# NCAR/icar

Measured on AMD Instinct MI355X. Metric: grid-cell updates/sec (advection+microphysics), higher is better.
Workload: dtype f32; 1 GPU; 512x512x40 global grid, mpdata order-2+FCT advection of 9 scalars + thompson microphysics, ideal hill case (SURVEY 8d); decomposition=1x1, backend=none, ranks_seen=1, halo_check=not applicable (one image, no process group), mpdata_arithmetic=fused kernel (<= 1e-5 of the local scale per step)

## Files before the change

### icar_amd/csrc/ctx.h

```cpp
#pragma once
#include <hip/hip_runtime.h>
#include <string>
#include <map>
#include <vector>
#include "../../include/icar_hip.h"

#define ICAR_MAX_ADV 12

struct Dims {
    int nx, nz, ny;
    int sk, sj;
    __host__ __device__ inline int idx(int i, int k, int j) const { return i + nx * (k + nz * j); }
};

struct VarPtrs { float *p[ICAR_MAX_ADV]; };
struct CVarPtrs { const float *p[ICAR_MAX_ADV]; };

struct TimingGroup { double total_ms = 0; int launches = 0; };

struct ThompsonTables;
struct LinWinds;
struct Wsm3State;
struct Wsm6State;
struct IcarComm;


struct IcarStepState {
    bool configured = false;
    icar_hip_step_config cfg;
    std::vector<float> dz_levels;
    double model_time = 0.0;
    double mp_last_model_time = -999.0;
    int winds_scheme = 0, winds_dens = 0; float winds_dt = 0.f;
    float *h_val = nullptr;
    bool early_open = false, early_wreal = false, early_face = false;
    bool failed = false;
    bool winds_first = true;
};

enum { MPC_AU = 0, MPC_CUV, MPC_CUW, MPC_AV, MPC_CVU, MPC_CVW, MPC_AW, MPC_CWU, MPC_CWV, MPC_GH, MPC_GV, MPC_N };

struct icar_hip_ctx {
    int device = 0;
    int ims, ime, kms, kme, jms, jme;
    Dims d;
    size_t n3 = 0;
    hipStream_t stream = nullptr;
    bool own_stream = false;
    hipStream_t aux = nullptr, main_saved = nullptr;
    hipEvent_t ev_fork = nullptr, ev_join = nullptr;
    bool on_aux = false;
    void *field[ICAR_N_FIELDS] = {nullptr};
    float *dqdt[ICAR_N_FIELDS] = {nullptr};
    float *U = nullptr, *V = nullptr, *W = nullptr, *Wdz = nullptr;
    float *mpc = nullptr;
    int mpc_dens = -1;
    float *alt[ICAR_N_ADVECTABLE] = {nullptr};
    float *mpx_buf = nullptr;
    int mpx_nv = 0;
    int mpdata_exact = 0;
    bool winds_valid = false;
    unsigned long long wind_version = 0;
    bool wind_ptr_escaped = false;
    struct { bool valid = false, reduced = false; unsigned long long ver = 0; float dx = 0.f; std::vector<float> dzl; } cfl_pre;
    float *h_cfl_pre = nullptr;
    bool cfl_wait_failed = false;
    hipEvent_t cfl_ev = nullptr;
    float *iw_adj = nullptr;
    float *wgr_tmp = nullptr;
    float *d_red = nullptr;
    std::vector<float> dzl_host;
    int *d_flag = nullptr;
    ThompsonTables *thompson = nullptr;
    LinWinds *linwinds = nullptr;
    Wsm3State *wsm3 = nullptr;
    Wsm6State *wsm6 = nullptr;
    IcarComm *comm = nullptr;
    IcarStepState step;
    bool timing = false;
    std::string timing_only;
    std::vector<hipEvent_t> event_pool;
    std::map<std::string, TimingGroup> timers;
    std::vector<std::pair<std::string, std::pair<hipEvent_t, hipEvent_t>>> pending;
};

void icar_set_error(const std::string &msg);
int icar_hip_check(hipError_t e, const char *what);
#define HIPCHK(x) do { if (icar_hip_check((x), #x)) return 1; } while (0)

size_t icar_field_count(const icar_hip_ctx *c, int field);
float *icar_field_f(icar_hip_ctx *c, int field, bool required = true);

struct ScopedTimer {
    icar_hip_ctx *c; const char *group; hipEvent_t e0 = nullptr, e1 = nullptr;
    ScopedTimer(icar_hip_ctx *c_, const char *g);
    ~ScopedTimer();
};

int icar_advect_setup_winds(icar_hip_ctx *c, int scheme, float dt, float dx, int advect_density, bool with_wreal = false, bool *wreal_done = nullptr);
int icar_advect_run(icar_hip_ctx *c, int scheme, int order, int fct, int advect_density, const int *fields, int n);
int icar_mp_simple_run(icar_hip_ctx *c, float dt, int its, int ite, int jts, int jte, int kts, int kte, int *err);
int icar_mp_simple_run_tiles(icar_hip_ctx *c, float dt, int ntiles, const int tiles[][4], int kts, int kte, int *err);
int icar_mp_run(icar_hip_ctx *c, double dt_in, int halo, int subset);
int icar_update_dt(icar_hip_ctx *c, double *seconds);
int icar_substep(icar_hip_ctx *c, double dt, bool enforce);
int icar_halo_pack(icar_hip_ctx *c, int dir, int halo, const int *fields, int n, float *buf, bool unpack);
int icar_halo_pack_dirs(icar_hip_ctx *c, int ndir, const int *dirs, int halo, const int *fields, int n, void *const *bufs, bool unpack);
int icar_max_courant_run(icar_hip_ctx *c, float dx, const float *dz_levels, float *out, float *d_out);
int icar_max_abs_winds_run(icar_hip_ctx *c, float *out3);
int icar_balance_uvw_run(icar_hip_ctx *c, float dx, int update);
int icar_iterative_winds_correct_w(icar_hip_ctx *c, int update);
int icar_mass_conservative_acceleration(icar_hip_ctx *c, int update);
int icar_iterative_winds_sweep(icar_hip_ctx *c, float dx, int nsweeps, int update);
int icar_make_winds_grid_relative(icar_hip_ctx *c, int update);
int icar_box_copy(icar_hip_ctx *c, int field, int which, int i0, int ni, int j0, int nj, float *buf, bool unpack);
enum { ICAR_DIAG_CELL = 4, ICAR_DIAG_FACE = 8 };
int icar_diagnostic_update_run(icar_hip_ctx *c, int parts);
int icar_max_courant_prefetch_run(icar_hip_ctx *c, float dx, const float *dz_levels, bool allreduce);
bool icar_cfl_prefetched_global(icar_hip_ctx *c, float dx, const float *dz_levels, float *value);
bool icar_cfl_prefetch_waiting(icar_hip_ctx *c);
inline void icar_winds_changed(icar_hip_ctx *c) { c->winds_valid = false; ++c->wind_version; }
int icar_apply_forcing_run(icar_hip_ctx *c, double dt, const int *fields, const int *fb, int n, int w, int e, int s, int nn);
int icar_enforce_limits_run(icar_hip_ctx *c, const int *fields, int n);
int icar_thompson_init_run(icar_hip_ctx *c, const float *params, const int *flags);
int icar_thompson_run(icar_hip_ctx *c, float dt, int its, int ite, int jts, int jte, int kts, int kte,
                      int ids, int ide, int jds, int jde, int kds, int kde);
int icar_thompson_run_tiles(icar_hip_ctx *c, float dt, int ntiles, const int (*tiles)[4], int kts, int kte,
                            int ids, int ide, int jds, int jde, int kds, int kde);
int icar_thompson_prepare_constants(icar_hip_ctx *c);
void icar_thompson_free(icar_hip_ctx *c);
void icar_linwinds_free(icar_hip_ctx *c);
void icar_wsm3_free(icar_hip_ctx *c);
int icar_wsm3_init_run(icar_hip_ctx *c);
int icar_wsm3_run(icar_hip_ctx *c, float dt, int its, int ite, int jts, int jte, int kts, int kte);
void icar_wsm6_free(icar_hip_ctx *c);
int icar_wsm6_init_run(icar_hip_ctx *c);
int icar_wsm6_run(icar_hip_ctx *c, float dt, int its, int ite, int jts, int jte, int kts, int kte);
int icar_wsm6_run_tiles(icar_hip_ctx *c, float dt, int ntiles, const int tiles[][4], int kts, int kte);
int icar_linwinds_setup_run(icar_hip_ctx *c, const icar_hip_lt_options *o, const float *terrain, int nxg, int nyg, int ids, int jds, float dx);
int icar_linear_perturbation_run(icar_hip_ctx *c, float U, float V, float Nsq, float zb, float zt, float minimum_step, double *u_out, double *v_out);
int icar_linwinds_build_lut_run(icar_hip_ctx *c, const float *zb, const float *zt, int nlev);
int icar_linwinds_build_lut_varying_run(icar_hip_ctx *c, const float *zb3, const float *zt3, int nlev);
int icar_linwinds_lut_copy(icar_hip_ctx *c, int comp, float *host, int to_dev);
int icar_linwinds_lut_entry(icar_hip_ctx *c, int comp, int k, int i, int j, float *host);
int icar_linwinds_pert_copy(icar_hip_ctx *c, int comp, float *host, int to_dev);
int icar_linwinds_terrain_frequency(icar_hip_ctx *c, double *out, size_t cap, int *fnx, int *fny);
int icar_spatial_winds_run(icar_hip_ctx *c, int update);
int icar_thompson_table_download(icar_hip_ctx *c, const char *name, double *out, size_t cap, size_t *n_out);
```

### icar_amd/csrc/mpdata.hip

```cpp
#include "ctx.h"
#include <algorithm>
#include <cmath>
#include <type_traits>

#define MP_HL 3
#define MP_XOUT (64 - 2 * MP_HL)
#define MP_NW 8
#define MP_KB 5
#define MP_ZH 2
#define EPSQ 1e-10f
#define EPSF 1e-15f
#define HEPSQ 0.5e-10f

__device__ __forceinline__ float dpp_l(float x)
{ return __int_as_float(__builtin_amdgcn_mov_dpp(__float_as_int(x), 0x138, 0xf, 0xf, true)); }
__device__ __forceinline__ float dpp_r(float x)
{ return __int_as_float(__builtin_amdgcn_mov_dpp(__float_as_int(x), 0x130, 0xf, 0xf, true)); }
__device__ __forceinline__ float dpp_l2(float x, float o)
{ return __int_as_float(__builtin_amdgcn_update_dpp(__float_as_int(o), __float_as_int(x), 0x138, 0xf, 0xf, true)); }
__device__ __forceinline__ float dpp_r2(float x, float o)
{ return __int_as_float(__builtin_amdgcn_update_dpp(__float_as_int(o), __float_as_int(x), 0x130, 0xf, 0xf, true)); }
__device__ __forceinline__ float opaque(float x) { asm volatile("" : "+v"(x)); return x; }
__device__ __forceinline__ float frcp(float x) { return __builtin_amdgcn_rcpf(x); }
__device__ __forceinline__ float upw(float l, float r, float U) { return U * (U > 0.0f ? l : r); }
__device__ __forceinline__ float exact_quot(float a, float g, float &r)
{
    const float r0 = frcp(g);
    r = __builtin_fmaf(__builtin_fmaf(-g, r0, 1.0f), r0, r0);
    const float y = opaque(a * r);
    return __builtin_fmaf(__builtin_fmaf(-g, y, a), r, y);
}
__device__ __forceinline__ float max3f(float a, float b, float c) { return fmaxf(fmaxf(a, b), c); }
__device__ __forceinline__ float min3f(float a, float b, float c) { return fminf(fminf(a, b), c); }
using rsrc_t = __amdgpu_buffer_rsrc_t;
__device__ __forceinline__ rsrc_t mkrsrc(const float *p) { return __builtin_amdgcn_make_buffer_rsrc((void *)p, 0, -1, 0x00020000); }
__device__ __forceinline__ float ldb(rsrc_t r, int voff, int soff) { return __builtin_bit_cast(float, __builtin_amdgcn_raw_buffer_load_b32(r, voff, soff, 0)); }
__device__ __forceinline__ void stb(rsrc_t r, int voff, int soff, float v) { __builtin_amdgcn_raw_buffer_store_b32(__builtin_bit_cast(int, v), r, voff, soff, 0); }
template <bool RHO>
__global__ void __launch_bounds__(256)
k_mpdata_coef(Dims d, const float *__restrict__ U, const float *__restrict__ V, const float *__restrict__ Wz, const float *__restrict__ rho,
              const float *__restrict__ jaco, const float *__restrict__ dz, float *__restrict__ C)
{
    const size_t n3 = (size_t)d.nx * d.nz * d.ny;
    const int i = blockIdx.x * 64 + threadIdx.x, k = blockIdx.y * 4 + threadIdx.y, j = blockIdx.z;
    if (i >= d.nx || k >= d.nz) return;
    const int nx = d.nx, nz = d.nz, ny = d.ny;
    const int iL = max(i - 1, 0), iR = min(i + 1, nx - 1), jP = max(j - 1, 0), jN = min(j + 1, ny - 1), kB = max(k - 1, 0), kT = min(k + 1, nz - 1);
    auto at = [&](int ii, int kk, int jj) { return ii + nx * (kk + nz * jj); };
    auto G = [&](int ii, int kk, int jj) { const int c = at(ii, kk, jj); return RHO ? jaco[c] * rho[c] : jaco[c]; };
    const int c = at(i, k, j);
    const bool xin = (i > 0) && (i < nx - 1), kin = (k > 0) && (k < nz - 1);
    const float g = G(i, k, j), dzc = dz[c];
    {
        const float rG = frcp(g + G(iL, k, j));
        const float evv = (V[c] + V[at(i, k, jN)]) + (V[at(iL, k, j)] + V[at(iL, k, jN)]);
        const float evw = (Wz[c] + Wz[at(i, kB, j)]) + (Wz[at(iL, k, j)] + Wz[at(iL, kB, j)]);
        const float Uc = U[c], aU = fabsf(Uc), c0 = 0.0625f * Uc * rG;
        C[MPC_AU * n3 + c] = 0.5f * aU * (1.0f - 2.0f * aU * rG); C[MPC_CUV * n3 + c] = c0 * evv; C[MPC_CUW * n3 + c] = kin ? c0 * evw : 0.0f;
    }
    {
        const float rG = frcp(g + G(i, k, jP));
        const float evu = (U[at(i, k, jP)] + U[c]) + (U[at(iR, k, jP)] + U[at(iR, k, j)]);
        const float evw = (Wz[at(i, k, jP)] + Wz[at(i, kB, jP)]) + (Wz[c] + Wz[at(i, kB, j)]);
        const float Vc = V[c], aV = fabsf(Vc), c0 = 0.0625f * Vc * rG;
        C[MPC_AV * n3 + c] = 0.5f * aV * (1.0f - 2.0f * aV * rG); C[MPC_CVU * n3 + c] = xin ? c0 * evu : 0.0f; C[MPC_CVW * n3 + c] = kin ? c0 * evw : 0.0f;
    }
    if (k < nz - 1) {
        const float rG = frcp(g + G(i, kT, j));
        const float evu = (U[c] + U[at(i, kT, j)]) + (U[at(iR, k, j)] + U[at(iR, kT, j)]);
        const float evv = (V[c] + V[at(i, k, jN)]) + (V[at(i, kT, j)] + V[at(i, kT, jN)]);
        const float Wc = Wz[c], aW = fabsf(Wc), c0 = 0.0625f * Wc * rG;
        C[MPC_AW * n3 + c] = 0.5f * aW * (1.0f - 2.0f * aW * rG) * dzc; C[MPC_CWU * n3 + c] = xin ? c0 * evu * dzc : 0.0f; C[MPC_CWV * n3 + c] = c0 * evv * dzc;
    } else { C[MPC_AW * n3 + c] = 0.f; C[MPC_CWU * n3 + c] = 0.f; C[MPC_CWV * n3 + c] = 0.f; }
    const float gh = g, gv = RHO ? (dzc * jaco[c]) * rho[c] : dzc * jaco[c];
    C[MPC_GH * n3 + c] = gh; C[MPC_GV * n3 + c] = gv;
}

template <bool ST, int PAR> struct MpMode { static constexpr bool steady = ST; static constexpr int par = PAR; };

template <int KB, bool FCT, bool PASS1, bool EXACT>
__global__ void __launch_bounds__(64 * MP_NW) __attribute__((amdgpu_num_vgpr(124)))
k_mpdata_fused(Dims d, CVarPtrs qin, VarPtrs qout,
               const float *__restrict__ Ug, const float *__restrict__ Vg, const float *__restrict__ Wg,
               const float *__restrict__ Cg, unsigned asz, int clen, int ntile, int nchunk, int nscal, int nkr, int kstore)
{
    constexpr int H = KB + 2;
    __shared__ float s_q2[2][MP_NW][2][64];
    __shared__ float s_bz[2][MP_NW][4][64];
    constexpr int NW2 = MP_NW + 2;
    __shared__ int s_sync[3 * NW2 + 64];
    constexpr int NA4 = (H + 3) / 4, NB4 = 2 * KB;
    __shared__ float4 s_park[NA4 + NB4][64 * MP_NW];
    constexpr int NG4 = (KB + 3) / 4;
    __shared__ float4 s_rv[2][NG4][64 * MP_NW];

    const int lane = threadIdx.x;
    const int wv = __builtin_amdgcn_readfirstlane(threadIdx.y), nw = blockDim.y;
    const int tid = lane + 64 * wv;
    const int nx = d.nx, nz = d.nz, ny = d.ny;
    const int sj4 = 4 * d.sj;
    int tile, chunk, m, kr;
    {
        const unsigned id = blockIdx.x, nv = (unsigned)nscal, nitem = (unsigned)(ntile * nchunk * nkr) * nv;
        const unsigned cap = (nitem + 7u) / 8u, xcd = id & 7u, slot = id >> 3;
        const unsigned it = xcd * cap + slot;
        if (slot >= cap || it >= nitem) return;
        for (int t = tid; t < 2 * NW2; t += 64 * nw) { const int j = t % NW2; s_sync[t] = (j == 0 || j > nw) ? 0x7fffffff : 0; }
        __syncthreads();
        const unsigned g = it / nv;
        m = (int)(it - g * nv);
        tile = (int)(g % (unsigned)ntile); chunk = (int)((g / (unsigned)ntile) % (unsigned)nchunk); kr = (int)(g / (unsigned)(ntile * nchunk));
    }
    const int ka = kr * kstore, kb = min(ka + kstore - 1, nz - 1), kbase = max(ka - MP_ZH, 0);
    const float *__restrict__ qp = qin.p[0];
    float *__restrict__ outp = qout.p[0];
#pragma unroll
    for (int mm = 1; mm < ICAR_MAX_ADV; ++mm) if (mm == m) { qp = qin.p[mm]; outp = qout.p[mm]; }
    const rsrc_t q = mkrsrc(qp), out = mkrsrc(outp), Ur = mkrsrc(Ug), Vr = mkrsrc(Vg), Wr = mkrsrc(Wg),
                 cr = mkrsrc(Cg);

    const int i = 1 - MP_HL + tile * MP_XOUT + lane;
    const int ic = min(max(i, 0), nx - 1);
    const bool xin = (i > 0) && (i < nx - 1), xring = (i == 0) || (i == nx - 1);
    const bool lane_store = ((lane >= MP_HL) && (lane < 64 - MP_HL) && xin) || xring;
    float rm = (i <= 0 || i >= nx - 1) ? 0.0f : 1.0f;
    const int ja = 1 + chunk * clen, jb = min(ja + clen - 1, ny - 2);
    const int k0 = kbase + wv * KB;
    int vk[H];
#pragma unroll
    for (int h = 0; h < H; ++h) { vk[h] = 4 * ic + min(max(k0 - 1 + h, 0), nz - 1) * nx * 4; asm volatile("" : "+v"(vk[h])); }
    asm volatile("" : "+v"(rm));
    const float gmul = __int_as_float(__builtin_amdgcn_readfirstlane((k0 == 0) ? 0 : 0x3f800000));
    const bool topwave = (k0 + KB == nz);
    const int htop_u = __builtin_amdgcn_readfirstlane(nz - k0), kst0_u = __builtin_amdgcn_readfirstlane(ka - k0), kst1_u = __builtin_amdgcn_readfirstlane(kb - k0);
    const int wlo = max(wv - 1, 0), whi = min(wv + 1, nw - 1);
    const int q2lo = (wv > 0) ? 1 : 0, q2hi = (wv < nw - 1) ? 0 : 1;
    const int bzlo = (wv > 0) ? 2 : 0, bzhi = (wv < nw - 1) ? 0 : 2;
    int *const fpost = (lane == 0) ? &s_sync[1 + wv] : &s_sync[2 * NW2 + lane];
    int seqA = 0, seqB = 0;
#define MP_POST(e, seq)                                                                                                   \
    {                                                                                                                      \
        ++seq;                                                                                                             \
        __hip_atomic_store(fpost + (e) * NW2, seq, __ATOMIC_RELEASE, __HIP_MEMORY_SCOPE_WORKGROUP);                         \
    }
#define MP_WAIT(e, seq)                                                                                                    \
    {                                                                                                                      \
        int spin = 0;                                                                                                      \
        for (;;) {                                                                                                         \
            const int fa = __hip_atomic_load(&s_sync[(e) * NW2 + wv], __ATOMIC_ACQUIRE, __HIP_MEMORY_SCOPE_WORKGROUP);      \
            const int fb = __hip_atomic_load(&s_sync[(e) * NW2 + wv + 2], __ATOMIC_ACQUIRE, __HIP_MEMORY_SCOPE_WORKGROUP);  \
            if (__builtin_amdgcn_readfirstlane(min(fa, fb)) >= seq) break;                                                 \
            __builtin_amdgcn_s_sleep(1);                                                                                   \
            if (++spin > (1 << 26)) __builtin_trap();                        \
        }                                                                                                                  \
    }

#define LDQ(h, po) ldb(q, vk[h], (po))
#define LDC(a, h, po) ldb(cr, vk[h], (int)((unsigned)(a) * asz + (unsigned)(po)))
#define CLAMPJ(p) min(max((p), 0), ny - 1)

    struct QBuf { float v[H]; };
    struct PSet {
        float q2[H];
        float m[KB], n[KB];
        float Dx[KB], Sx[KB], Dz[KB], Sz[KB];
        float Fyd[KB];
        float rh[KB];
        float mh0, nh0, mh1, nh1;
    };
    QBuf Q0, Q1;
    PSet S0, S1;
#pragma unroll
    for (int kk = 0; kk < KB; ++kk) { S0.m[kk] = S0.n[kk] = 0.f; S0.Dx[kk] = S0.Sx[kk] = S0.Dz[kk] = S0.Sz[kk] = 0.f; S0.Fyd[kk] = 0.f; S0.rh[kk] = 0.f; }
#pragma unroll
    for (int h = 0; h < H; ++h) S0.q2[h] = 0.f;
    S0.mh0 = 0.f; S0.nh0 = 0.f; S0.mh1 = 0.f; S0.nh1 = 0.f;
    S1 = S0;
#pragma unroll
    for (int t = 0; t < NA4 + NB4; ++t) s_park[t][tid] = make_float4(0.f, 0.f, 0.f, 0.f);
#pragma unroll
    for (int t = 0; t < 2 * NG4; ++t) s_rv[t / NG4][t % NG4][tid] = make_float4(0.f, 0.f, 0.f, 0.f);
    const int P0 = ja - 3;
    float WN[KB + 1], UN[KB], VNN[KB], ghN[KB], gvN[KB];
#define ISSUE_LOADS_A(oN_, oNN_)                                                                                         \
    {                                                                                                                    \
        _Pragma("unroll") for (int h = 0; h <= KB; ++h) WN[h] = ldb(Wr, vk[h], (oN_));                                   \
        _Pragma("unroll") for (int kk = 0; kk < KB; ++kk) { UN[kk] = ldb(Ur, vk[kk + 1], (oN_)); VNN[kk] = ldb(Vr, vk[kk + 1], (oNN_)); } \
        _Pragma("unroll") for (int kk = 0; kk < KB; ++kk) { ghN[kk] = LDC(MPC_GH, kk + 1, (oN_)); gvN[kk] = LDC(MPC_GV, kk + 1, (oN_)); } \
    }
    {
        const int o0 = CLAMPJ(P0) * sj4, o1 = CLAMPJ(P0 + 1) * sj4, o2 = CLAMPJ(P0 + 2) * sj4;
        float qP0[KB], V1[KB];
#pragma unroll
        for (int kk = 0; kk < KB; ++kk) { qP0[kk] = LDQ(kk + 1, o0); V1[kk] = ldb(Vr, vk[kk + 1], o1); }
#pragma unroll
        for (int h = 0; h < H; ++h) Q0.v[h] = LDQ(h, o1);
#pragma unroll
        for (int h = 0; h < H; ++h) Q1.v[h] = LDQ(h, o2);
        ISSUE_LOADS_A(o1, o2)
        if (PASS1) {
#pragma unroll
            for (int kk = 0; kk < KB; ++kk) S0.Fyd[kk] = opaque(upw(qP0[kk], Q0.v[kk + 1], V1[kk]));
        }
    }
    auto step = [&](auto md, QBuf &qN, QBuf &qNN, PSet &sP, PSet &sN, const int P) {
        constexpr bool STEADY = decltype(md)::steady;
        const int par = STEADY ? decltype(md)::par : ((P - P0) & 1);
        const int N = P + 1;
        const bool haveN = STEADY || ((N >= 0) && (N <= ny - 1));
        const int oP = (STEADY ? P : CLAMPJ(P)) * sj4, oN = (STEADY ? N : CLAMPJ(N)) * sj4;
        int htop = htop_u, kst0 = kst0_u, kst1 = kst1_u;
        if (!EXACT) asm volatile("" : "+s"(htop), "+s"(kst0), "+s"(kst1));
        float avN[KB], cvuN[KB], cvwN[KB], auP[KB], cuvP[KB], cuwP[KB];
#pragma unroll
        for (int kk = 0; kk < KB; ++kk) { avN[kk] = LDC(MPC_AV, kk + 1, oN); cvuN[kk] = LDC(MPC_CVU, kk + 1, oN); cvwN[kk] = LDC(MPC_CVW, kk + 1, oN); }
#pragma unroll
        for (int kk = 0; kk < KB; ++kk) { auP[kk] = LDC(MPC_AU, kk + 1, oP); cuvP[kk] = LDC(MPC_CUV, kk + 1, oP); cuwP[kk] = LDC(MPC_CUW, kk + 1, oP); }
        __builtin_amdgcn_sched_barrier(0);

        float *const q2N = sN.q2;
        const float *const q2P = sP.q2;
        float v2N[KB], FyN[KB], rvN[KB];
#pragma unroll
        for (int kk = 0; kk < KB; ++kk) { v2N[kk] = 0.f; FyN[kk] = 0.f; rvN[kk] = 0.f; }
        auto yface = [&](const int kk) {
            const int h = kk + 1;
            const float t = avN[kk] * (q2N[h] - q2P[h]) * frcp(q2N[h] + q2P[h] + EPSQ)
                          - cvuN[kk] * (sN.Dx[kk] + sP.Dx[kk]) * frcp(sN.Sx[kk] + sP.Sx[kk])
                          - cvwN[kk] * (sN.Dz[kk] + sP.Dz[kk]) * frcp(sN.Sz[kk] + sP.Sz[kk]);
            v2N[kk] = t; FyN[kk] = upw(q2P[h], q2N[h], t);
        };
        if (haveN) {
            if (PASS1) {
                const float rmN = (STEADY || (N > 0 && N < ny - 1)) ? rm : 0.0f;
                float FzT[KB + 1];
#pragma unroll
                for (int h = 0; h <= KB; ++h) FzT[h] = opaque(upw(qN.v[h], qN.v[h + 1], WN[h]));
                FzT[0] *= gmul;
                auto donor = [&](const int kk) {
                    const int h = kk + 1;
                    const float FxL = opaque(upw(dpp_l(qN.v[h]), qN.v[h], UN[kk])), FxR = dpp_r(FxL);
                    const float Fn = opaque(upw(qN.v[h], qNN.v[h], VNN[kk]));
                    const float dh = ((FxR - FxL) + (Fn - sP.Fyd[kk])) * rmN, dv = (FzT[h] - FzT[h - 1]) * rmN;
                    const float t = qN.v[h] - exact_quot(dh, ghN[kk], sN.rh[kk]);
                    q2N[h] = t - exact_quot(dv, gvN[kk], rvN[kk]);
                    sN.Fyd[kk] = Fn;
                };
                donor(0);
                if (KB > 1) donor(KB - 1);
                s_q2[par][wv][0][lane] = q2N[1]; s_q2[par][wv][1][lane] = q2N[KB];
                MP_POST(0, seqA)
#pragma unroll
                for (int kk = 1; kk < KB - 1; ++kk) donor(kk);
            } else {
#pragma unroll
                for (int h = 0; h < H; ++h) q2N[h] = qN.v[h];
#pragma unroll
                for (int kk = 0; kk < KB; ++kk) { sN.rh[kk] = frcp(ghN[kk]); rvN[kk] = frcp(gvN[kk]); }
            }
#pragma unroll
            for (int kk = 0; kk < KB; ++kk) { sN.m[kk] = fmaxf(q2N[kk + 1], qN.v[kk + 1]); sN.n[kk] = fminf(q2N[kk + 1], qN.v[kk + 1]); }
#pragma unroll
            for (int kk = 0; kk < KB; ++kk) {
                const int h = kk + 1;
                const float l = dpp_l(q2N[h]);
                sN.Dx[kk] = dpp_r(q2N[h]) - l; sN.Sx[kk] = dpp_r2(q2N[h], l) + (l + HEPSQ);
                if (kk > 0 && kk < KB - 1) { sN.Dz[kk] = q2N[h + 1] - q2N[h - 1]; sN.Sz[kk] = q2N[h + 1] + (q2N[h - 1] + HEPSQ); }
            }
            if (PASS1) {
                MP_WAIT(0, seqA)
                q2N[0] = s_q2[par][wlo][q2lo][lane];
                q2N[H - 1] = s_q2[par][whi][q2hi][lane];
            }
            sN.Dz[0] = q2N[2] - q2N[0]; sN.Sz[0] = q2N[2] + (q2N[0] + HEPSQ);
            if (KB > 1) { sN.Dz[KB - 1] = q2N[KB + 1] - q2N[KB - 1]; sN.Sz[KB - 1] = q2N[KB + 1] + (q2N[KB - 1] + HEPSQ); }
            sN.mh0 = fmaxf(q2N[0], qN.v[0]); sN.nh0 = fminf(q2N[0], qN.v[0]);
            sN.mh1 = fmaxf(q2N[H - 1], qN.v[H - 1]); sN.nh1 = fminf(q2N[H - 1], qN.v[H - 1]);
        } else {
#pragma unroll
            for (int h = 0; h < H; ++h) q2N[h] = qN.v[h];
#pragma unroll
            for (int kk = 0; kk < KB; ++kk) { sN.m[kk] = sN.n[kk] = 0.f; sN.Dx[kk] = sN.Sx[kk] = sN.Dz[kk] = sN.Sz[kk] = 0.f; sN.Fyd[kk] = 0.f; sN.rh[kk] = 0.f; }
            sN.mh0 = 0.f; sN.nh0 = 0.f; sN.mh1 = 0.f; sN.nh1 = 0.f;
        }

        {
            float pv[NG4 * 4];
#pragma unroll
            for (int t = 0; t < NG4 * 4; ++t) pv[t] = (t < KB) ? rvN[t < KB ? t : 0] : 0.f;
#pragma unroll
            for (int t = 0; t < NG4; ++t) s_rv[par][t][tid] = make_float4(pv[4 * t], pv[4 * t + 1], pv[4 * t + 2], pv[4 * t + 3]);
        }
        __builtin_amdgcn_sched_barrier(0);
        float awP[KB + 1], cwuP[KB + 1], cwvP[KB + 1];
#pragma unroll
        for (int h = 0; h <= KB; ++h) { awP[h] = LDC(MPC_AW, h, oP); cwuP[h] = LDC(MPC_CWU, h, oP); cwvP[h] = LDC(MPC_CWV, h, oP); }
        {
            const int o3 = (STEADY ? P + 3 : CLAMPJ(P + 3)) * sj4;
            if (STEADY) {
#pragma unroll
                for (int h = 0; h < H; ++h) qN.v[h] = LDQ(h, o3);
            } else {
                qN = qNN;
#pragma unroll
                for (int h = 0; h < H; ++h) qNN.v[h] = LDQ(h, o3);
            }
        }
        __builtin_amdgcn_sched_barrier(0);

        if (STEADY || (P >= 0 && haveN)) {
#pragma unroll
            for (int kk = 0; kk < KB; ++kk) yface(kk);
        }

        float bYin[KB], bYout[KB], FyLimS[KB], outM[KB];
        auto ylim = [&]() {
#pragma unroll
        for (int kk = 0; kk < KB; ++kk) {
            const int h = kk + 1;
            const float4 pa = s_park[NA4 + 2 * kk][tid], pb = s_park[NA4 + 2 * kk + 1][tid];
            const float mM = pa.x, nM = pa.y, v2S = pa.z, FyS = pa.w, bYinM = pb.x, bYoutM = pb.y, acc = pb.z, rdhM = pb.w;
            if (FCT) {
                const float qc = q2P[h];
                float qmax = max3f(mM, sP.m[kk], sN.m[kk]), qmin = min3f(nM, sP.n[kk], sN.n[kk]);
                float fin = fmaxf(0.f, FyS) - fminf(0.f, FyN[kk]), fout = fmaxf(0.f, FyN[kk]) - fminf(0.f, FyS);
                if (!STEADY && P <= 0) { qmax = fmaxf(sP.m[kk], sN.m[kk]); qmin = fminf(sP.n[kk], sN.n[kk]); fin = 0.f; fout = 0.f; }
                if (!STEADY && P >= ny - 1) { qmax = fmaxf(mM, qc); qmin = fminf(nM, qc); fin = 0.f; fout = 0.f; }
                bYin[kk] = (qmax - qc) * frcp(fin + EPSF); bYout[kk] = (qc - qmin) * frcp(fout + EPSF);
                const float s = fminf(1.0f, (v2S > 0.0f) ? fminf(bYin[kk], bYoutM) : fminf(bYinM, bYout[kk]));
                FyLimS[kk] = s * FyS;
            } else { bYin[kk] = bYout[kk] = 0.f; FyLimS[kk] = FyS; }
            outM[kk] = acc - FyLimS[kk] * rdhM;
        }
        };
        float xdiv[KB], zdiv[KB];
#pragma unroll
        for (int kk = 0; kk < KB; ++kk) { xdiv[kk] = zdiv[kk] = 0.f; }
        float q2M[NA4 * 4];
#pragma unroll
        for (int t = 0; t < NA4; ++t) { const float4 v = s_park[t][tid]; q2M[4 * t] = v.x; q2M[4 * t + 1] = v.y; q2M[4 * t + 2] = v.z; q2M[4 * t + 3] = v.w; }
        const bool planeP = STEADY || ((P >= ja) && (P <= jb));
        if (planeP) {
            float Dy[H], Sy[H];
#pragma unroll
            for (int h = 0; h < H; ++h) { Dy[h] = q2N[h] - q2M[h]; Sy[h] = q2N[h] + (q2M[h] + HEPSQ); }
            float Fx[KB], u2[KB];
#pragma unroll
            for (int kk = 0; kk < KB; ++kk) {
                const int h = kk + 1;
                const float qL = dpp_l(q2P[h]);
                const float t = auP[kk] * (q2P[h] - qL) * frcp(q2P[h] + qL + EPSQ)
                              - cuvP[kk] * (Dy[h] + dpp_l(Dy[h])) * frcp(Sy[h] + dpp_l(Sy[h]))
                              - cuwP[kk] * (sP.Dz[kk] + dpp_l(sP.Dz[kk])) * frcp(sP.Sz[kk] + dpp_l(sP.Sz[kk]));
                u2[kk] = t; Fx[kk] = upw(qL, q2P[h], t);
            }
            float DxA[H], SxA[H];
#pragma unroll
            for (int kk = 0; kk < KB; ++kk) { DxA[kk + 1] = sP.Dx[kk]; SxA[kk + 1] = sP.Sx[kk]; }
            { const float l0 = dpp_l(q2P[0]), l1 = dpp_l(q2P[H - 1]);
              DxA[0] = dpp_r(q2P[0]) - l0; SxA[0] = dpp_r2(q2P[0], l0) + (l0 + HEPSQ);
              DxA[H - 1] = dpp_r(q2P[H - 1]) - l1; SxA[H - 1] = dpp_r2(q2P[H - 1], l1) + (l1 + HEPSQ); }
            float Fz[KB + 1], w2[KB + 1];
#pragma unroll
            for (int hf = 0; hf <= KB; ++hf) {
                float t = awP[hf] * (q2P[hf + 1] - q2P[hf]) * frcp(q2P[hf + 1] + q2P[hf] + EPSQ)
                        - cwuP[hf] * (DxA[hf] + DxA[hf + 1]) * frcp(SxA[hf] + SxA[hf + 1])
                        - cwvP[hf] * (Dy[hf] + Dy[hf + 1]) * frcp(Sy[hf] + Sy[hf + 1]);
                if (hf == 0) t *= gmul;
                w2[hf] = t; Fz[hf] = upw(q2P[hf], q2P[hf + 1], t);
            }
            float FxLim[KB];
#pragma unroll
            for (int kk = 0; kk < KB; ++kk) {
                const int h = kk + 1;
                if (FCT) {
                    const float qc = q2P[h], Fp = fmaxf(0.f, Fx[kk]), Fm = fminf(0.f, Fx[kk]);
                    const float fin = Fp - dpp_r(Fm), fout = dpp_r(Fp) - Fm;
                    const float qmax = fmaxf(dpp_r(sP.m[kk]), opaque(fmaxf(dpp_l(sP.m[kk]), sP.m[kk])));
                    const float qmin = fminf(dpp_r(sP.n[kk]), opaque(fminf(dpp_l(sP.n[kk]), sP.n[kk])));
                    const float bin = (qmax - qc) * frcp(__builtin_fmaf(fin, rm, EPSF)), bout = (qc - qmin) * frcp(__builtin_fmaf(fout, rm, EPSF));
                    const float bLin = dpp_l(bin), bLout = dpp_l(bout);
                    const float s = fminf(1.0f, (u2[kk] > 0.0f) ? fminf(bin, bLout) : fminf(bLin, bout));
                    FxLim[kk] = s * Fx[kk];
                } else FxLim[kk] = Fx[kk];
                xdiv[kk] = dpp_r(FxLim[kk]) - FxLim[kk];
            }
            float FzLim[KB + 1];
            if (FCT) {
                float bZin[H], bZout[H], Fzp[KB + 1], Fzm[KB + 1];
#pragma unroll
                for (int hf = 0; hf <= KB; ++hf) { Fzp[hf] = fmaxf(0.f, Fz[hf]); Fzm[hf] = fminf(0.f, Fz[hf]); }
                auto betaz = [&](const int kk) {
                    const int h = kk + 1;
                    const float qc = q2P[h];
                    float FzTp = Fzp[h], FzTm = Fzm[h];
                    const float mlo = (kk > 0) ? sP.m[kk - 1] : sP.mh0, nlo = (kk > 0) ? sP.n[kk - 1] : sP.nh0;
                    float mhi = (kk < KB - 1) ? sP.m[kk + 1] : sP.mh1, nhi = (kk < KB - 1) ? sP.n[kk + 1] : sP.nh1;
                    float mc = sP.m[kk], nc = sP.n[kk];
                    if (EXACT ? (h == KB) : true) {
                        const bool tp = EXACT ? topwave : (h >= htop);
                        mc = tp ? qc : mc; nc = tp ? qc : nc; mhi = tp ? qc : mhi; nhi = tp ? qc : nhi; FzTp = tp ? Fzp[h - 1] : FzTp; FzTm = tp ? Fzm[h - 1] : FzTm;
                    }
                    const float qmax = max3f(mlo, mc, mhi), qmin = min3f(nlo, nc, nhi);
                    const float fin = Fzp[h - 1] - FzTm, fout = FzTp - Fzm[h - 1];
                    bZin[h] = (qmax - qc) * frcp(fin + EPSF); bZout[h] = (qc - qmin) * frcp(fout + EPSF);
                };
                betaz(0);
                if (KB > 1) betaz(KB - 1);
                s_bz[par][wv][0][lane] = bZin[1]; s_bz[par][wv][1][lane] = bZout[1]; s_bz[par][wv][2][lane] = bZin[KB]; s_bz[par][wv][3][lane] = bZout[KB];
                MP_POST(1, seqB)
#pragma unroll
                for (int kk = 1; kk < KB - 1; ++kk) betaz(kk);
#pragma unroll
                for (int hf = 1; hf < KB; ++hf) {
                    const float s = fminf(1.0f, (w2[hf] > 0.0f) ? fminf(bZin[hf + 1], bZout[hf]) : fminf(bZin[hf], bZout[hf + 1]));
                    FzLim[hf] = s * Fz[hf];
                }
                MP_WAIT(1, seqB)
                bZin[0] = s_bz[par][wlo][bzlo][lane]; bZout[0] = s_bz[par][wlo][bzlo + 1][lane];
                bZin[H - 1] = s_bz[par][whi][bzhi][lane]; bZout[H - 1] = s_bz[par][whi][bzhi + 1][lane];
#pragma unroll
                for (int hf = 0; hf <= KB; hf += KB) {
                    const float s = fminf(1.0f, (w2[hf] > 0.0f) ? fminf(bZin[hf + 1], bZout[hf]) : fminf(bZin[hf], bZout[hf + 1]));
                    FzLim[hf] = s * Fz[hf];
                }
            } else {
#pragma unroll
                for (int hf = 0; hf <= KB; ++hf) FzLim[hf] = Fz[hf];
            }
#pragma unroll
            for (int kk = 0; kk < KB; ++kk) zdiv[kk] = FzLim[kk + 1] - FzLim[kk];
        }

        __builtin_amdgcn_sched_barrier(0);
        {
            const int o2 = (STEADY ? P + 2 : CLAMPJ(P + 2)) * sj4, o3 = (STEADY ? P + 3 : CLAMPJ(P + 3)) * sj4;
            ISSUE_LOADS_A(o2, o3)
        }
        __builtin_amdgcn_sched_barrier(0);

        ylim();

        const int M = P - 1;
        if (STEADY || (M >= ja && M <= jb)) {
            if (lane_store) {
#pragma unroll
                for (int kk = 0; kk < KB; ++kk)
                    if (EXACT || (kk >= kst0 && kk <= kst1)) stb(out, vk[kk + 1], M * sj4, outM[kk]);
            }
        }
        if (!STEADY && M == 0 && ja == 1) {
#pragma unroll
            for (int kk = 0; kk < KB; ++kk)
                if (lane_store && (EXACT || (kk >= kst0 && kk <= kst1))) stb(out, vk[kk + 1], 0, q2M[kk + 1]);
        }
        if (!STEADY && P == ny - 1 && jb == ny - 2) {
#pragma unroll
            for (int kk = 0; kk < KB; ++kk)
                if (lane_store && (EXACT || (kk >= kst0 && kk <= kst1))) stb(out, vk[kk + 1], (ny - 1) * sj4, q2P[kk + 1]);
        }
        const float rmP = (STEADY || (P > 0 && P < ny - 1)) ? rm : 0.0f;
        float rvP[NG4 * 4];
#pragma unroll
        for (int t = 0; t < NG4; ++t) { const float4 v = s_rv[par ^ 1][t][tid]; rvP[4 * t] = v.x; rvP[4 * t + 1] = v.y; rvP[4 * t + 2] = v.z; rvP[4 * t + 3] = v.w; }
#pragma unroll
        for (int kk = 0; kk < KB; ++kk) {
            const int h = kk + 1;
            const float rdh = sP.rh[kk] * rmP, rdv = rvP[kk] * rmP;
            const float accP = q2P[h] - (xdiv[kk] - FyLimS[kk]) * rdh - zdiv[kk] * rdv;
            s_park[NA4 + 2 * kk][tid] = make_float4(sP.m[kk], sP.n[kk], v2N[kk], FyN[kk]);
            s_park[NA4 + 2 * kk + 1][tid] = make_float4(bYin[kk], bYout[kk], accP, rdh);
        }
        {
            float pq[NA4 * 4];
#pragma unroll
            for (int t = 0; t < NA4 * 4; ++t) pq[t] = (t < H) ? q2P[t < H ? t : 0] : 0.f;
#pragma unroll
            for (int t = 0; t < NA4; ++t) s_park[t][tid] = make_float4(pq[4 * t], pq[4 * t + 1], pq[4 * t + 2], pq[4 * t + 3]);
        }
        if (!STEADY) sP = sN;
    };
    using MdGeneric = MpMode<false, 0>; using MdEven = MpMode<true, 0>; using MdOdd = MpMode<true, 1>;
    {
        const int s0 = ja + 1, s1 = max(min(jb + 1, ny - 4), s0 - 1);
        const int npair = (s1 - s0 + 1) / 2, s1p = s0 + 2 * npair - 1;
        for (int ph = 0; ph < 2; ++ph) {
            const int lo = ph ? s1p + 1 : P0, hi = ph ? jb + 1 : s0 - 1;
            for (int P = lo; P <= hi; ++P) step(MdGeneric{}, Q0, Q1, S0, S1, P);
            if (ph == 0)
                for (int P = s0; P < s1p; P += 2) { step(MdEven{}, Q0, Q1, S0, S1, P); step(MdOdd{}, Q1, Q0, S1, S0, P + 1); }
        }
    }
#undef ISSUE_LOADS_A
#undef LDQ
#undef LDC
#undef MP_POST
#undef MP_WAIT
#undef CLAMPJ
}

template <int KB>
static void launch_fused(icar_hip_ctx *c, bool fct, bool pass1, bool exact, const CVarPtrs &in, const VarPtrs &out, int nv,
                         int nw, int clen, int ntile, int nchunk, int nkr, int kstore)
{
    const unsigned nitem = (unsigned)(ntile * nchunk * nkr * nv), cap = (nitem + 7u) / 8u;
    const dim3 g(8u * cap), b(64, nw);
#define GO(F, P1, E) hipLaunchKernelGGL((k_mpdata_fused<KB, F, P1, E>), g, b, 0, c->stream, c->d, in, out, c->U, c->V, c->W, c->mpc, (unsigned)(c->n3 * sizeof(float)), clen, ntile, nchunk, nv, nkr, kstore)
#define GO2(F, P1) { if (exact) GO(F, P1, true); else GO(F, P1, false); }
    if (fct) { if (pass1) GO2(true, true) else GO2(true, false) } else { if (pass1) GO2(false, true) else GO2(false, false) }
#undef GO2
#undef GO
}

int icar_mpdata_coef_run(icar_hip_ctx *c, bool rho_on)
{
    const float *jaco = icar_field_f(c, ICAR_F_JACOBIAN), *dz = icar_field_f(c, ICAR_F_ADVECTION_DZ);
    const float *rho = rho_on ? icar_field_f(c, ICAR_F_DENSITY) : nullptr;
    if (!jaco || !dz || (rho_on && !rho)) return 1;
    if (c->n3 * sizeof(float) * MPC_N >= ((size_t)1 << 32)) { icar_set_error("mpdata: a tile of more than 97 M cells is not supported (32-bit buffer offsets into the coefficient arrays)"); return 1; }
    if (!c->mpc) HIPCHK(hipMalloc(&c->mpc, c->n3 * sizeof(float) * MPC_N));
    const dim3 g((c->d.nx + 63) / 64, (c->d.nz + 3) / 4, c->d.ny), b(64, 4);
    if (rho_on) hipLaunchKernelGGL(k_mpdata_coef<true>, g, b, 0, c->stream, c->d, c->U, c->V, c->Wdz, rho, jaco, dz, c->mpc);
    else        hipLaunchKernelGGL(k_mpdata_coef<false>, g, b, 0, c->stream, c->d, c->U, c->V, c->Wdz, rho, jaco, dz, c->mpc);
    HIPCHK(hipGetLastError());
    c->mpc_dens = rho_on ? 1 : 0;
    return 0;
}

int icar_mpdata_fused_run(icar_hip_ctx *c, bool rho_on, bool fct, bool pass1, const CVarPtrs &in, const VarPtrs &out, int nv)
{
    const int nx = c->d.nx, nz = c->d.nz, ny = c->d.ny;
    if (!c->mpc || c->mpc_dens != (rho_on ? 1 : 0)) { icar_set_error("mpdata: icar_hip_setup_winds(scheme 2) with the same advect_density must come first"); return 1; }
    if (nx < 3 || ny < 3) { icar_set_error("mpdata: tile must be at least 3 x 3 cells"); return 1; }
    if ((size_t)nx * nz * ny * sizeof(float) >= ((size_t)1 << 31)) { icar_set_error("mpdata: a field of 2 GiB or more is not supported (32-bit buffer offsets)"); return 1; }
    const int ntile = std::max(1, (nx - 2 + MP_XOUT - 1) / MP_XOUT);
    const int cap_lv = MP_NW * MP_KB;
    int nkr = 1;
    while (nkr * cap_lv - 2 * MP_ZH * (nkr - 1) < nz) ++nkr;
    const int kstore = (nz + nkr - 1) / nkr;
    const int blk_lv = std::min(nz, kstore + (nkr > 1 ? 2 * MP_ZH : 0));
    const int kb = (blk_lv + MP_NW - 1) / MP_NW, nw = (blk_lv + kb - 1) / kb;
    const int rows = ny - 2, per = ntile * nkr * nv;
    int nchunk = 1; double best = -1.0;
    for (int n = 1; n <= std::max(1, rows / 16); ++n) {
        const int cl = (rows + n - 1) / n, nn = (rows + cl - 1) / cl;
        const double items = (double)per * nn, rounds = std::ceil(items / 256.0);
        const double eff = items / (256.0 * rounds) * cl / (cl + 3.5);
        if (eff > best + 1e-9) { best = eff; nchunk = nn; }
    }
    const int clen = (rows + nchunk - 1) / nchunk;
    nchunk = (rows + clen - 1) / clen;
    const bool exact = (nkr == 1) && (kb * nw == nz);
#define KBCASE(K) case K: launch_fused<K>(c, fct, pass1, exact, in, out, nv, nw, clen, ntile, nchunk, nkr, kstore); break;
    switch (kb) { KBCASE(1) KBCASE(2) KBCASE(3) KBCASE(4) KBCASE(5) default: icar_set_error("mpdata: internal level-range error"); return 1; }
#undef KBCASE
    HIPCHK(hipGetLastError());
    return 0;
}
```

Before: 3.858 billion grid-cell updates/s.

## Interleave MPDATA coefficients into AoS tuples and pack GH/GV/U/W into float4

The coefficient buffer moves from eleven separate planar arrays to per-direction triples (x, y, z) stored interleaved per cell, plus a 256-byte-aligned float4 array holding gh, gv, U and W. The fused advection kernel now reads these with single 96-bit and 128-bit buffer loads in place of many scalar loads, and no longer reads U directly. This is meant to cut the number of memory instructions and improve locality in the bandwidth-bound kernel. In exchange the coefficient kernel does strided 3-wide stores and must copy U and W into the buffer, which also lowers the maximum supported tile size.

```diff
diff --git a/icar_amd/csrc/ctx.h b/icar_amd/csrc/ctx.h
--- a/icar_amd/csrc/ctx.h
+++ b/icar_amd/csrc/ctx.h
@@ -39,6 +39,8 @@
 };
 
 enum { MPC_AU = 0, MPC_CUV, MPC_CUW, MPC_AV, MPC_CVU, MPC_CVW, MPC_AW, MPC_CWU, MPC_CWV, MPC_GH, MPC_GV, MPC_N };
+__host__ __device__ inline size_t mpc_cell_bytes(size_t n3) { return (MPC_GH * n3 * sizeof(float) + 255) & ~(size_t)255; }
+__host__ __device__ inline size_t mpc_bytes(size_t n3) { return mpc_cell_bytes(n3) + 4 * n3 * sizeof(float); }
 
 struct icar_hip_ctx {
     int device = 0;
diff --git a/icar_amd/csrc/mpdata.hip b/icar_amd/csrc/mpdata.hip
--- a/icar_amd/csrc/mpdata.hip
+++ b/icar_amd/csrc/mpdata.hip
@@ -33,13 +33,18 @@
 __device__ __forceinline__ float max3f(float a, float b, float c) { return fmaxf(fmaxf(a, b), c); }
 __device__ __forceinline__ float min3f(float a, float b, float c) { return fminf(fminf(a, b), c); }
 using rsrc_t = __amdgpu_buffer_rsrc_t;
+typedef unsigned u32x3 __attribute__((ext_vector_type(3)));
+typedef unsigned u32x4 __attribute__((ext_vector_type(4)));
 __device__ __forceinline__ rsrc_t mkrsrc(const float *p) { return __builtin_amdgcn_make_buffer_rsrc((void *)p, 0, -1, 0x00020000); }
 __device__ __forceinline__ float ldb(rsrc_t r, int voff, int soff) { return __builtin_bit_cast(float, __builtin_amdgcn_raw_buffer_load_b32(r, voff, soff, 0)); }
+__device__ __forceinline__ u32x3 ldb3(rsrc_t r, int voff, int soff) { return __builtin_amdgcn_raw_buffer_load_b96(r, voff, soff, 0); }
+__device__ __forceinline__ u32x4 ldb4(rsrc_t r, int voff, int soff) { return __builtin_amdgcn_raw_buffer_load_b128(r, voff, soff, 0); }
+__device__ __forceinline__ float fu(unsigned x) { return __uint_as_float(x); }
 __device__ __forceinline__ void stb(rsrc_t r, int voff, int soff, float v) { __builtin_amdgcn_raw_buffer_store_b32(__builtin_bit_cast(int, v), r, voff, soff, 0); }
 template <bool RHO>
 __global__ void __launch_bounds__(256)
-k_mpdata_coef(Dims d, const float *__restrict__ U, const float *__restrict__ V, const float *__restrict__ Wz, const float *__restrict__ rho,
-              const float *__restrict__ jaco, const float *__restrict__ dz, float *__restrict__ C)
+k_mpdata_coef(Dims d, const float *__restrict__ U, const float *__restrict__ V, const float *__restrict__ Wz, const float *__restrict__ W,
+              const float *__restrict__ rho, const float *__restrict__ jaco, const float *__restrict__ dz, float *__restrict__ C)
 {
     const size_t n3 = (size_t)d.nx * d.nz * d.ny;
     const int i = blockIdx.x * 64 + threadIdx.x, k = blockIdx.y * 4 + threadIdx.y, j = blockIdx.z;
@@ -51,29 +56,30 @@
     const int c = at(i, k, j);
     const bool xin = (i > 0) && (i < nx - 1), kin = (k > 0) && (k < nz - 1);
     const float g = G(i, k, j), dzc = dz[c];
+    float *const Cx = C + 3 * (size_t)c, *const Cy = Cx + 3 * n3, *const Cz = Cx + 6 * n3;
     {
         const float rG = frcp(g + G(iL, k, j));
         const float evv = (V[c] + V[at(i, k, jN)]) + (V[at(iL, k, j)] + V[at(iL, k, jN)]);
         const float evw = (Wz[c] + Wz[at(i, kB, j)]) + (Wz[at(iL, k, j)] + Wz[at(iL, kB, j)]);
         const float Uc = U[c], aU = fabsf(Uc), c0 = 0.0625f * Uc * rG;
-        C[MPC_AU * n3 + c] = 0.5f * aU * (1.0f - 2.0f * aU * rG); C[MPC_CUV * n3 + c] = c0 * evv; C[MPC_CUW * n3 + c] = kin ? c0 * evw : 0.0f;
+        Cx[0] = 0.5f * aU * (1.0f - 2.0f * aU * rG); Cx[1] = c0 * evv; Cx[2] = kin ? c0 * evw : 0.0f;
     }
     {
         const float rG = frcp(g + G(i, k, jP));
         const float evu = (U[at(i, k, jP)] + U[c]) + (U[at(iR, k, jP)] + U[at(iR, k, j)]);
         const float evw = (Wz[at(i, k, jP)] + Wz[at(i, kB, jP)]) + (Wz[c] + Wz[at(i, kB, j)]);
         const float Vc = V[c], aV = fabsf(Vc), c0 = 0.0625f * Vc * rG;
-        C[MPC_AV * n3 + c] = 0.5f * aV * (1.0f - 2.0f * aV * rG); C[MPC_CVU * n3 + c] = xin ? c0 * evu : 0.0f; C[MPC_CVW * n3 + c] = kin ? c0 * evw : 0.0f;
+        Cy[0] = 0.5f * aV * (1.0f - 2.0f * aV * rG); Cy[1] = xin ? c0 * evu : 0.0f; Cy[2] = kin ? c0 * evw : 0.0f;
     }
     if (k < nz - 1) {
         const float rG = frcp(g + G(i, kT, j));
         const float evu = (U[c] + U[at(i, kT, j)]) + (U[at(iR, k, j)] + U[at(iR, kT, j)]);
         const float evv = (V[c] + V[at(i, k, jN)]) + (V[at(i, kT, j)] + V[at(i, kT, jN)]);
         const float Wc = Wz[c], aW = fabsf(Wc), c0 = 0.0625f * Wc * rG;
-        C[MPC_AW * n3 + c] = 0.5f * aW * (1.0f - 2.0f * aW * rG) * dzc; C[MPC_CWU * n3 + c] = xin ? c0 * evu * dzc : 0.0f; C[MPC_CWV * n3 + c] = c0 * evv * dzc;
-    } else { C[MPC_AW * n3 + c] = 0.f; C[MPC_CWU * n3 + c] = 0.f; C[MPC_CWV * n3 + c] = 0.f; }
+        Cz[0] = 0.5f * aW * (1.0f - 2.0f * aW * rG) * dzc; Cz[1] = xin ? c0 * evu * dzc : 0.0f; Cz[2] = c0 * evv * dzc;
+    } else { Cz[0] = 0.f; Cz[1] = 0.f; Cz[2] = 0.f; }
     const float gh = g, gv = RHO ? (dzc * jaco[c]) * rho[c] : dzc * jaco[c];
-    C[MPC_GH * n3 + c] = gh; C[MPC_GV * n3 + c] = gv;
+    ((float4 *)((char *)C + mpc_cell_bytes(n3)))[c] = make_float4(gh, gv, U[c], W[c]);
 }
 
 template <bool ST, int PAR> struct MpMode { static constexpr bool steady = ST; static constexpr int par = PAR; };
@@ -81,8 +87,8 @@
 template <int KB, bool FCT, bool PASS1, bool EXACT>
 __global__ void __launch_bounds__(64 * MP_NW) __attribute__((amdgpu_num_vgpr(124)))
 k_mpdata_fused(Dims d, CVarPtrs qin, VarPtrs qout,
-               const float *__restrict__ Ug, const float *__restrict__ Vg, const float *__restrict__ Wg,
-               const float *__restrict__ Cg, unsigned asz, int clen, int ntile, int nchunk, int nscal, int nkr, int kstore)
+               const float *__restrict__ Vg, const float *__restrict__ Wg,
+               const float *__restrict__ Cg, unsigned fsz, unsigned cbase, int clen, int ntile, int nchunk, int nscal, int nkr, int kstore)
 {
     constexpr int H = KB + 2;
     __shared__ float s_q2[2][MP_NW][2][64];
@@ -116,7 +122,7 @@
     float *__restrict__ outp = qout.p[0];
 #pragma unroll
     for (int mm = 1; mm < ICAR_MAX_ADV; ++mm) if (mm == m) { qp = qin.p[mm]; outp = qout.p[mm]; }
-    const rsrc_t q = mkrsrc(qp), out = mkrsrc(outp), Ur = mkrsrc(Ug), Vr = mkrsrc(Vg), Wr = mkrsrc(Wg),
+    const rsrc_t q = mkrsrc(qp), out = mkrsrc(outp), Vr = mkrsrc(Vg), Wr = mkrsrc(Wg),
                  cr = mkrsrc(Cg);
 
     const int i = 1 - MP_HL + tile * MP_XOUT + lane;
@@ -156,7 +162,10 @@
     }
 
 #define LDQ(h, po) ldb(q, vk[h], (po))
-#define LDC(a, h, po) ldb(cr, vk[h], (int)((unsigned)(a) * asz + (unsigned)(po)))
+#define VK3(h) ([&] { int t_ = vk[h]; asm volatile("" : "+v"(t_)); return 3 * t_; }())
+#define VK4(h) ([&] { int t_ = vk[h]; asm volatile("" : "+v"(t_)); return 4 * t_; }())
+#define LDF(f, v3, po) ldb3(cr, (v3), (int)((unsigned)(f) * fsz + 3u * (unsigned)(po)))
+#define LDG(v4, po) ldb4(cr, (v4), (int)(cbase + 4u * (unsigned)(po)))
 #define CLAMPJ(p) min(max((p), 0), ny - 1)
 
     struct QBuf { float v[H]; };
@@ -184,9 +193,12 @@
     float WN[KB + 1], UN[KB], VNN[KB], ghN[KB], gvN[KB];
 #define ISSUE_LOADS_A(oN_, oNN_)                                                                                         \
     {                                                                                                                    \
-        _Pragma("unroll") for (int h = 0; h <= KB; ++h) WN[h] = ldb(Wr, vk[h], (oN_));                                   \
-        _Pragma("unroll") for (int kk = 0; kk < KB; ++kk) { UN[kk] = ldb(Ur, vk[kk + 1], (oN_)); VNN[kk] = ldb(Vr, vk[kk + 1], (oNN_)); } \
-        _Pragma("unroll") for (int kk = 0; kk < KB; ++kk) { ghN[kk] = LDC(MPC_GH, kk + 1, (oN_)); gvN[kk] = LDC(MPC_GV, kk + 1, (oN_)); } \
+        WN[0] = ldb(Wr, vk[0], (oN_));                                                                                   \
+        _Pragma("unroll") for (int kk = 0; kk < KB; ++kk) {                                                              \
+            const u32x4 g_ = LDG(VK4(kk + 1), (oN_));                                                                    \
+            ghN[kk] = fu(g_.x); gvN[kk] = fu(g_.y); UN[kk] = fu(g_.z); WN[kk + 1] = fu(g_.w);                             \
+        }                                                                                                                \
+        _Pragma("unroll") for (int kk = 0; kk < KB; ++kk) VNN[kk] = ldb(Vr, vk[kk + 1], (oNN_));                         \
     }
     {
         const int o0 = CLAMPJ(P0) * sj4, o1 = CLAMPJ(P0 + 1) * sj4, o2 = CLAMPJ(P0 + 2) * sj4;
@@ -213,9 +225,11 @@
         if (!EXACT) asm volatile("" : "+s"(htop), "+s"(kst0), "+s"(kst1));
         float avN[KB], cvuN[KB], cvwN[KB], auP[KB], cuvP[KB], cuwP[KB];
 #pragma unroll
-        for (int kk = 0; kk < KB; ++kk) { avN[kk] = LDC(MPC_AV, kk + 1, oN); cvuN[kk] = LDC(MPC_CVU, kk + 1, oN); cvwN[kk] = LDC(MPC_CVW, kk + 1, oN); }
-#pragma unroll
-        for (int kk = 0; kk < KB; ++kk) { auP[kk] = LDC(MPC_AU, kk + 1, oP); cuvP[kk] = LDC(MPC_CUV, kk + 1, oP); cuwP[kk] = LDC(MPC_CUW, kk + 1, oP); }
+        for (int kk = 0; kk < KB; ++kk) {
+            const int v3 = VK3(kk + 1);
+            const u32x3 a = LDF(1, v3, oN), b = LDF(0, v3, oP);
+            avN[kk] = fu(a.x); cvuN[kk] = fu(a.y); cvwN[kk] = fu(a.z); auP[kk] = fu(b.x); cuvP[kk] = fu(b.y); cuwP[kk] = fu(b.z);
+        }
         __builtin_amdgcn_sched_barrier(0);
 
         float *const q2N = sN.q2;
@@ -294,7 +308,7 @@
         __builtin_amdgcn_sched_barrier(0);
         float awP[KB + 1], cwuP[KB + 1], cwvP[KB + 1];
 #pragma unroll
-        for (int h = 0; h <= KB; ++h) { awP[h] = LDC(MPC_AW, h, oP); cwuP[h] = LDC(MPC_CWU, h, oP); cwvP[h] = LDC(MPC_CWV, h, oP); }
+        for (int h = 0; h <= KB; ++h) { const u32x3 z = LDF(2, VK3(h), oP); awP[h] = fu(z.x); cwuP[h] = fu(z.y); cwvP[h] = fu(z.z); }
         {
             const int o3 = (STEADY ? P + 3 : CLAMPJ(P + 3)) * sj4;
             if (STEADY) {
@@ -493,7 +507,10 @@
     }
 #undef ISSUE_LOADS_A
 #undef LDQ
-#undef LDC
+#undef LDF
+#undef LDG
+#undef VK3
+#undef VK4
 #undef MP_POST
 #undef MP_WAIT
 #undef CLAMPJ
@@ -505,7 +522,7 @@
 {
     const unsigned nitem = (unsigned)(ntile * nchunk * nkr * nv), cap = (nitem + 7u) / 8u;
     const dim3 g(8u * cap), b(64, nw);
-#define GO(F, P1, E) hipLaunchKernelGGL((k_mpdata_fused<KB, F, P1, E>), g, b, 0, c->stream, c->d, in, out, c->U, c->V, c->W, c->mpc, (unsigned)(c->n3 * sizeof(float)), clen, ntile, nchunk, nv, nkr, kstore)
+#define GO(F, P1, E) hipLaunchKernelGGL((k_mpdata_fused<KB, F, P1, E>), g, b, 0, c->stream, c->d, in, out, c->V, c->W, c->mpc, (unsigned)(3 * c->n3 * sizeof(float)), (unsigned)mpc_cell_bytes(c->n3), clen, ntile, nchunk, nv, nkr, kstore)
 #define GO2(F, P1) { if (exact) GO(F, P1, true); else GO(F, P1, false); }
     if (fct) { if (pass1) GO2(true, true) else GO2(true, false) } else { if (pass1) GO2(false, true) else GO2(false, false) }
 #undef GO2
@@ -517,11 +534,11 @@
     const float *jaco = icar_field_f(c, ICAR_F_JACOBIAN), *dz = icar_field_f(c, ICAR_F_ADVECTION_DZ);
     const float *rho = rho_on ? icar_field_f(c, ICAR_F_DENSITY) : nullptr;
     if (!jaco || !dz || (rho_on && !rho)) return 1;
-    if (c->n3 * sizeof(float) * MPC_N >= ((size_t)1 << 32)) { icar_set_error("mpdata: a tile of more than 97 M cells is not supported (32-bit buffer offsets into the coefficient arrays)"); return 1; }
-    if (!c->mpc) HIPCHK(hipMalloc(&c->mpc, c->n3 * sizeof(float) * MPC_N));
+    if (mpc_bytes(c->n3) >= ((size_t)1 << 32)) { icar_set_error("mpdata: a tile of more than 82 M cells is not supported (32-bit buffer offsets into the coefficient tuples)"); return 1; }
+    if (!c->mpc) HIPCHK(hipMalloc(&c->mpc, mpc_bytes(c->n3)));
     const dim3 g((c->d.nx + 63) / 64, (c->d.nz + 3) / 4, c->d.ny), b(64, 4);
-    if (rho_on) hipLaunchKernelGGL(k_mpdata_coef<true>, g, b, 0, c->stream, c->d, c->U, c->V, c->Wdz, rho, jaco, dz, c->mpc);
-    else        hipLaunchKernelGGL(k_mpdata_coef<false>, g, b, 0, c->stream, c->d, c->U, c->V, c->Wdz, rho, jaco, dz, c->mpc);
+    if (rho_on) hipLaunchKernelGGL(k_mpdata_coef<true>, g, b, 0, c->stream, c->d, c->U, c->V, c->Wdz, c->W, rho, jaco, dz, c->mpc);
+    else        hipLaunchKernelGGL(k_mpdata_coef<false>, g, b, 0, c->stream, c->d, c->U, c->V, c->Wdz, c->W, rho, jaco, dz, c->mpc);
     HIPCHK(hipGetLastError());
     c->mpc_dens = rho_on ? 1 : 0;
     return 0;
```

New measurement: 3.952 billion grid-cell updates/s, median of 6. 2.4% higher.
